# mcveanlab/Corticall

Hardware: AMD Instinct MI355X
Metric: k-mers traversed/sec (whole node) + contigs/sec, k=47 3-color LdBG (higher is better)
Workload: dtype u64

## Files before the change

corticall_amd/csrc/rt.h:

```cpp
#pragma once
#include <stdint.h>
#include <stdlib.h>
#include <string.h>

#include <algorithm>
#include <map>
#include <mutex>
#include <string>
#include <type_traits>
#include <unordered_map>
#include <utility>
#include <vector>

#include "../../include/ldbg.h"
#include "ctx_host.h"

#ifndef LDBG_HOSTSIM
#include <hip/hip_runtime.h>
#define LDBG_KERNEL __global__
#define LDBG_WAVE_KERNEL __global__ __launch_bounds__(64)
#define LDBG_WAVE_KERNEL_N(n) __global__ __launch_bounds__(n)
#define LDBG_DEV __device__ __forceinline__
#define LDBG_HOSTDEV __host__ __device__ __forceinline__
#if defined(__HIP_DEVICE_COMPILE__)
// ... 4 lines not shown
#define LDBG_LDS(T, p) ((T*)(p))
#endif

namespace ldbg {
namespace rt {

inline void check(hipError_t e, const char* what) {
    if (e != hipSuccess) throw StatusError(LDBG_ERR_HIP, std::string(what) + ": " + hipGetErrorString(e));
}
inline int device_count() {
    int n = 0;
    hipError_t e = hipGetDeviceCount(&n);
    if (e != hipSuccess) { (void)hipGetLastError(); return 0; }
    return n;
}
inline void set_device(int d) { check(hipSetDevice(d), "hipSetDevice"); }
inline int cu_count(int d) {
    int n = 0;
    check(hipDeviceGetAttribute(&n, hipDeviceAttributeMultiprocessorCount, d), "hipDeviceGetAttribute");
    return n > 0 ? n : 256;
}
struct BlockCache {
    std::mutex m;
    std::unordered_map<void*, std::pair<int, size_t>> live;
    std::map<std::pair<int, size_t>, std::vector<void*>> free_;
    size_t held = 0;
    static size_t size_class(size_t n) {
        size_t c = 4096;
        while (c < n) { if (c + c / 2 >= n) return c + c / 2; c *= 2; }
        return c;
    }
    void release_all() {
        std::lock_guard<std::mutex> g(m);
        for (auto& kv : free_) for (void* p : kv.second) (void)hipFree(p);
        free_.clear(); held = 0;
    }
};
inline BlockCache& block_cache() { static BlockCache c; return c; }
inline void* dmalloc(size_t n) {
    void* p = nullptr;
    hipError_t e = hipMalloc(&p, n ? n : 1);
    if (e != hipSuccess) { (void)hipGetLastError(); block_cache().release_all(); e = hipMalloc(&p, n ? n : 1); }
    check(e, "hipMalloc");
    return p;
}
inline void dfree(void* p) {
    if (!p) return;
    { BlockCache& c = block_cache(); std::lock_guard<std::mutex> g(c.m); c.live.erase(p); }
    (void)hipFree(p);
}
inline void* tmalloc(size_t n) {
    BlockCache& c = block_cache();
    const size_t cls = BlockCache::size_class(n);
    if (cls > ((size_t)64 << 20)) return dmalloc(n);
    int dev = 0;
    check(hipGetDevice(&dev), "hipGetDevice");
    {
        std::lock_guard<std::mutex> g(c.m);
        auto it = c.free_.find({dev, cls});
        if (it != c.free_.end() && !it->second.empty()) {
            void* p = it->second.back();
            it->second.pop_back();
            c.held -= cls;
            c.live[p] = {dev, cls};
            return p;
        }
    }
    void* p = dmalloc(cls);
    std::lock_guard<std::mutex> g(c.m);
    c.live[p] = {dev, cls};
    return p;
}
inline void tfree(void* p) {
    if (!p) return;
    BlockCache& c = block_cache();
    {
        std::lock_guard<std::mutex> g(c.m);
        auto it = c.live.find(p);
        if (it != c.live.end() && c.held + it->second.second <= ((size_t)1 << 30)) {
            c.free_[it->second].push_back(p);
            c.held += it->second.second;
            c.live.erase(it);
            return;
        }
        if (it != c.live.end()) c.live.erase(it);
    }
    (void)hipFree(p);
}
inline void* hmalloc_pinned(size_t n) { void* p = nullptr; check(hipHostMalloc(&p, n ? n : 1, hipHostMallocDefault), "hipHostMalloc"); return p; }
inline void hfree_pinned(void* p) { if (p) (void)hipHostFree(p); }
inline bool host_is_pinned(const void* p) {
    hipPointerAttribute_t a;
    if (hipPointerGetAttributes(&a, p) != hipSuccess) { (void)hipGetLastError(); return false; }
    return a.type == hipMemoryTypeHost;
}
typedef hipStream_t stream_t;
inline stream_t stream_create() { hipStream_t s; check(hipStreamCreateWithFlags(&s, hipStreamNonBlocking), "hipStreamCreate"); return s; }
inline void stream_destroy(stream_t s) { if (s) (void)hipStreamDestroy(s); }
inline void stream_sync(stream_t s) { check(hipStreamSynchronize(s), "hipStreamSynchronize"); }
inline void h2d(void* d, const void* h, size_t n, stream_t s) { if (n) check(hipMemcpyAsync(d, h, n, hipMemcpyHostToDevice, s), "hipMemcpyAsync H2D"); }
inline void d2h(void* h, const void* d, size_t n, stream_t s) { if (n) check(hipMemcpyAsync(h, d, n, hipMemcpyDeviceToHost, s), "hipMemcpyAsync D2H"); }
inline void d2d(void* d, const void* s_, size_t n, stream_t s) { if (n) check(hipMemcpyAsync(d, s_, n, hipMemcpyDeviceToDevice, s), "hipMemcpyAsync D2D"); }
inline void dmemset(void* d, int v, size_t n, stream_t s) { if (n) check(hipMemsetAsync(d, v, n, s), "hipMemsetAsync"); }
inline void mem_info(size_t* free_b, size_t* total_b) { check(hipMemGetInfo(free_b, total_b), "hipMemGetInfo"); }
inline void launch_check(const char* name) { check(hipGetLastError(), name); }

struct Event {
    hipEvent_t e = nullptr;
    Event() { check(hipEventCreate(&e), "hipEventCreate"); }
    ~Event() { if (e) (void)hipEventDestroy(e); }
    Event(Event&& o) noexcept : e(o.e) { o.e = nullptr; }
    Event& operator=(Event&& o) noexcept { if (this != &o) { if (e) (void)hipEventDestroy(e); e = o.e; o.e = nullptr; } return *this; }
    Event(const Event&) = delete;
    Event& operator=(const Event&) = delete;
    void record(stream_t s) { check(hipEventRecord(e, s), "hipEventRecord"); }
    void wait() { check(hipEventSynchronize(e), "hipEventSynchronize"); }
    static float elapsed_ms(Event& a, Event& b) {
        check(hipEventSynchronize(b.e), "hipEventSynchronize");
        float ms = 0;
        check(hipEventElapsedTime(&ms, a.e, b.e), "hipEventElapsedTime");
        return ms;
    }
};

}
}

#define LDBG_LAUNCH(kernel, grid, block, stream, ...)                               \
    do {                                                                            \
        hipLaunchKernelGGL(kernel, dim3((unsigned)(grid)), dim3((unsigned)(block)), 0, stream, __VA_ARGS__); \
        ::ldbg::rt::launch_check(#kernel);                                          \
    } while (0)

namespace ldbg {
LDBG_DEV int64_t global_tid() { return (int64_t)blockIdx.x * blockDim.x + threadIdx.x; }
LDBG_DEV int64_t global_nthreads() { return (int64_t)gridDim.x * blockDim.x; }
LDBG_DEV unsigned long long atomic_add_u64(unsigned long long* p, unsigned long long v) { return atomicAdd(p, v); }
LDBG_DEV unsigned atomic_add_u32(unsigned* p, unsigned v) { return atomicAdd(p, v); }
LDBG_DEV unsigned atomic_min_u32(unsigned* p, unsigned v) { return atomicMin(p, v); }
LDBG_DEV unsigned atomic_or_u32(unsigned* p, unsigned v) { return atomicOr(p, v); }
LDBG_DEV unsigned long long atomic_min_u64(unsigned long long* p, unsigned long long v) { return atomicMin(p, v); }
LDBG_DEV unsigned long long atomic_cas_u64(unsigned long long* p, unsigned long long cmp, unsigned long long v) { return atomicCAS(p, cmp, v); }
LDBG_DEV unsigned long long atomic_exch_u64(unsigned long long* p, unsigned long long v) { return atomicExch(p, v); }
LDBG_DEV int wave_size() { return blockDim.x < 64u ? (int)blockDim.x : 64; }
LDBG_DEV int wave_lane() { return (int)(threadIdx.x & 63u); }
LDBG_DEV unsigned long long wave_ballot(bool p) { return __ballot(p ? 1 : 0); }
LDBG_DEV uint32_t wave_bcast_u32(uint32_t v, int src) { return (uint32_t)__builtin_amdgcn_readlane((int)v, __builtin_amdgcn_readfirstlane(src)); }
LDBG_DEV uint64_t wave_bcast_u64(uint64_t v, int src) {
    uint32_t lo = wave_bcast_u32((uint32_t)v, src), hi = wave_bcast_u32((uint32_t)(v >> 32), src);
    return ((uint64_t)hi << 32) | lo;
}
LDBG_DEV uint32_t wave_shfl_u32(uint32_t v, int src) { return (uint32_t)__shfl((int)v, src & 63, 64); }
LDBG_DEV uint64_t wave_shfl_u64(uint64_t v, int src) { return ((uint64_t)wave_shfl_u32((uint32_t)(v >> 32), src) << 32) | wave_shfl_u32((uint32_t)v, src); }
LDBG_DEV void wave_fence() { __threadfence_block(); }
LDBG_DEV void device_fence() { __threadfence(); }
LDBG_DEV uint64_t wave_shfl_xor_u64(uint64_t v, int m) {
    uint32_t lo = (uint32_t)__shfl_xor((int)(uint32_t)v, m, 64), hi = (uint32_t)__shfl_xor((int)(uint32_t)(v >> 32), m, 64);
    return ((uint64_t)hi << 32) | lo;
}
LDBG_DEV uint64_t wave_min_u64(uint64_t v) { for (int m = wave_size() >> 1; m > 0; m >>= 1) { uint64_t o = wave_shfl_xor_u64(v, m); v = o < v ? o : v; } return v; }
LDBG_DEV uint64_t wave_max_u64(uint64_t v) { for (int m = wave_size() >> 1; m > 0; m >>= 1) { uint64_t o = wave_shfl_xor_u64(v, m); v = o > v ? o : v; } return v; }
LDBG_DEV int wave_count_below(unsigned long long ballot) { return __builtin_popcountll(ballot & ((1ull << wave_lane()) - 1ull)); }
LDBG_DEV uint32_t wave_incl_scan_u32(uint32_t v) {
    const int lane = wave_lane();
    for (int d = 1; d < wave_size(); d <<= 1) { const uint32_t o = (uint32_t)__shfl_up((int)v, d, 64); if (lane >= d) v += o; }
    return v;
}
}

#else
#define LDBG_KERNEL static
#define LDBG_WAVE_KERNEL static
#define LDBG_WAVE_KERNEL_N(n) static
#define LDBG_DEV inline
#define LDBG_HOSTDEV inline
#define LDBG_GLOBAL(T, p) ((T*)(p))
#define LDBG_LDS(T, p) ((T*)(p))
#ifndef __forceinline__
#define __forceinline__
#endif

namespace ldbg {
namespace rt {
inline int device_count() { return 1; }
inline void set_device(int) {}
inline int cu_count(int) { return 256; }
inline bool poison() { static const bool on = getenv("LDBG_HOSTSIM_POISON") != nullptr; return on; }
inline void* dmalloc(size_t n) {
    if (!poison()) return calloc(n ? n : 1, 1);
    void* p = malloc(n ? n : 1);
    if (p) memset(p, 0xAB, n ? n : 1);
    return p;
}
inline void dfree(void* p) { free(p); }
inline void* tmalloc(size_t n) { return dmalloc(n); }
inline void tfree(void* p) { free(p); }
inline void* hmalloc_pinned(size_t n) { return malloc(n ? n : 1); }
inline void hfree_pinned(void* p) { free(p); }
inline bool host_is_pinned(const void*) { return getenv("LDBG_HOSTSIM_PAGEABLE") == nullptr; }
typedef void* stream_t;
inline stream_t stream_create() { return nullptr; }
inline void stream_destroy(stream_t) {}
inline void stream_sync(stream_t) {}
inline void h2d(void* d, const void* h, size_t n, stream_t) { if (n) memcpy(d, h, n); }
inline void d2h(void* h, const void* d, size_t n, stream_t) { if (n) memcpy(h, d, n); }
inline void d2d(void* d, const void* s, size_t n, stream_t) { if (n) memmove(d, s, n); }
inline void dmemset(void* d, int v, size_t n, stream_t) { if (n) memset(d, v, n); }
inline void mem_info(size_t* free_b, size_t* total_b) {
    size_t mb = 2048;
    if (const char* ev = getenv("LDBG_HOSTSIM_MEM_MB")) mb = (size_t)atoll(ev);
    *free_b = mb << 20; *total_b = mb << 20;
}
struct Event {
    void record(stream_t) {}
    void wait() {}
    static float elapsed_ms(Event&, Event&) { return 0.0f; }
};
}
}
#include <execinfo.h>
#include <ucontext.h>
#include <stdio.h>
#include <functional>
#include <vector>
namespace ldbg {
namespace sim {
struct Wave {
    int lanes = 1, cur = 0, live = 0, arrived = 0;
    unsigned long long gen = 0;
    bool active = false;
    ucontext_t sched;
    ucontext_t ctx[64];
    std::vector<char> stacks[64];
    uint8_t done[64];
    int kind[64];
    void* site[64];
    uint64_t x[2][64];
    uint64_t y[2][64];
    int64_t tid0 = 0, nthreads = 1;
    std::function<void()>* body = nullptr;
};
inline Wave& wave() { static thread_local Wave w; return w; }
inline int& lanes_setting() { static int n = [] { const char* e = getenv("LDBG_HOSTSIM_LANES"); int v = e ? atoi(e) : 1; return v < 1 ? 1 : (v > 64 ? 64 : v); }(); return n; }
inline int lanes_env() { return lanes_setting(); }
inline void yield() { Wave& w = wave(); swapcontext(&w.ctx[w.cur], &w.sched); }
inline int collective(int kind, uint64_t a, uint64_t b = 0) {
    Wave& w = wave();
    const int buf = (int)(w.gen & 1ull);
    const unsigned long long my_gen = w.gen;
    w.x[buf][w.cur] = a; w.y[buf][w.cur] = b; w.kind[w.cur] = kind; w.site[w.cur] = __builtin_return_address(0);
    w.arrived++;
    if (w.arrived == w.live) {
        for (int l = 0; l < w.lanes; l++)
            if (!w.done[l] && w.kind[l] != kind) {
                fprintf(stderr, "[hostsim] wavefront divergence: lane %d is at primitive %d (%p), lane %d at %d (%p); the arriving lane's stack:\n", w.cur, kind, w.site[w.cur], l, w.kind[l], w.site[l]);
                void* bt[32];
                backtrace_symbols_fd(bt, backtrace(bt, 32), 2);
                abort();
            }
        w.arrived = 0; w.gen++;
    } else {
        while (w.gen == my_gen) yield();
    }
    return buf;
}
inline void trampoline() {
    Wave& w = wave();
    (*w.body)();
    w.done[w.cur] = 1;
    w.live--;
    if (w.live > 0 && w.arrived == w.live) {
        const int kd = [&] { for (int l = 0; l < w.lanes; l++) if (!w.done[l]) return w.kind[l]; return 0; }();
        for (int l = 0; l < w.lanes; l++)
            if (!w.done[l] && w.kind[l] != kd) { fprintf(stderr, "[hostsim] wavefront divergence at a lane's exit\n"); abort(); }
        w.arrived = 0; w.gen++;
    }
    swapcontext(&w.ctx[w.cur], &w.sched);
}
void run_wave(int lanes, int64_t tid0, int64_t nthreads, std::function<void()>& body);
}
struct SimIdx { int64_t tid, nthreads; };
inline SimIdx& sim_idx() { static thread_local SimIdx s{0, 1}; return s; }
inline int64_t global_tid() { return sim_idx().tid; }
inline int64_t global_nthreads() { return sim_idx().nthreads; }
inline void sim::run_wave(int lanes, int64_t tid0, int64_t nthreads, std::function<void()>& body) {
    Wave& w = wave();
    w.lanes = lanes; w.live = lanes; w.arrived = 0; w.gen = 0; w.active = true; w.body = &body; w.tid0 = tid0; w.nthreads = nthreads;
    for (int l = 0; l < lanes; l++) {
        if (w.stacks[l].empty()) w.stacks[l].resize((size_t)1 << 20);
        w.done[l] = 0; w.kind[l] = 0;
        getcontext(&w.ctx[l]);
        w.ctx[l].uc_stack.ss_sp = w.stacks[l].data();
        w.ctx[l].uc_stack.ss_size = w.stacks[l].size();
        w.ctx[l].uc_link = &w.sched;
        makecontext(&w.ctx[l], (void (*)())sim::trampoline, 0);
    }
    while (w.live > 0) {
        for (int l = 0; l < lanes; l++) {
            if (w.done[l]) continue;
            w.cur = l;
            sim_idx().tid = tid0 + l; sim_idx().nthreads = nthreads;
            swapcontext(&w.sched, &w.ctx[l]);
        }
    }
    w.active = false; w.lanes = 1; w.cur = 0;
}
inline unsigned long long atomic_add_u64(unsigned long long* p, unsigned long long v) { unsigned long long o = *p; *p += v; return o; }
inline unsigned atomic_add_u32(unsigned* p, unsigned v) { unsigned o = *p; *p += v; return o; }
inline unsigned atomic_min_u32(unsigned* p, unsigned v) { unsigned o = *p; if (v < o) *p = v; return o; }
inline unsigned atomic_or_u32(unsigned* p, unsigned v) { unsigned o = *p; *p |= v; return o; }
inline unsigned long long atomic_min_u64(unsigned long long* p, unsigned long long v) { unsigned long long o = *p; if (v < o) *p = v; return o; }
inline unsigned long long atomic_cas_u64(unsigned long long* p, unsigned long long cmp, unsigned long long v) { unsigned long long o = *p; if (o == cmp) *p = v; return o; }
inline unsigned long long atomic_exch_u64(unsigned long long* p, unsigned long long v) { unsigned long long o = *p; *p = v; return o; }
inline int wave_size() { return sim::wave().active ? sim::wave().lanes : 1; }
inline int wave_lane() { return sim::wave().active ? sim::wave().cur : 0; }
inline unsigned long long wave_ballot(bool p) {
    sim::Wave& w = sim::wave();
    if (!w.active) return p ? 1ull : 0ull;
    const int b = sim::collective(1, p ? 1ull : 0ull);
    unsigned long long m = 0;
    for (int l = 0; l < w.lanes; l++) if (!w.done[l] && w.x[b][l]) m |= 1ull << l;
    return m;
}
inline uint64_t wave_shfl_u64(uint64_t v, int src) {
    sim::Wave& w = sim::wave();
    if (!w.active) return v;
    const int b = sim::collective(2, v);
    return w.x[b][src & (w.lanes - 1)];
}
inline uint32_t wave_shfl_u32(uint32_t v, int src) { return (uint32_t)wave_shfl_u64(v, src); }
inline uint32_t wave_bcast_u32(uint32_t v, int src) { return (uint32_t)wave_shfl_u64(v, src); }
inline uint64_t wave_bcast_u64(uint64_t v, int src) { return wave_shfl_u64(v, src); }
inline uint64_t wave_shfl_xor_u64(uint64_t v, int m) { return wave_shfl_u64(v, wave_lane() ^ m); }
inline void wave_fence() { if (sim::wave().active) (void)sim::collective(3, 0ull); }
inline void device_fence() {}
inline uint64_t wave_min_u64(uint64_t v) { for (int m = wave_size() >> 1; m > 0; m >>= 1) { uint64_t o = wave_shfl_xor_u64(v, m); v = o < v ? o : v; } return v; }
inline uint64_t wave_max_u64(uint64_t v) { for (int m = wave_size() >> 1; m > 0; m >>= 1) { uint64_t o = wave_shfl_xor_u64(v, m); v = o > v ? o : v; } return v; }
inline int wave_count_below(unsigned long long ballot) { return __builtin_popcountll(ballot & ((1ull << wave_lane()) - 1ull)); }
inline uint32_t wave_incl_scan_u32(uint32_t v) {
    sim::Wave& w = sim::wave();
    if (!w.active) return v;
    const int b = sim::collective(3, v);
    uint32_t s = 0;
    for (int l = 0; l <= w.cur; l++) if (!w.done[l]) s += (uint32_t)w.x[b][l];
    return s;
}
}

#define LDBG_LAUNCH(kernel, grid, block, stream, ...)                      \
    do {                                                                   \
        int64_t nt__ = (int64_t)(grid) * (int64_t)(block);                 \
        if (nt__ > 4096) nt__ = 4096;                                      \
        const int lanes__ = ::ldbg::sim::lanes_env() > 1 && (int64_t)(block) <= 64 ? (int)std::min<int64_t>((int64_t)(block), (int64_t)::ldbg::sim::lanes_env()) : 1; \
        if (lanes__ > 1) {                                                 \
            nt__ = (nt__ / lanes__) * lanes__; if (nt__ < lanes__) nt__ = lanes__; \
            std::function<void()> body__ = [&]() { kernel(__VA_ARGS__); }; \
            for (int64_t t__ = 0; t__ < nt__; t__ += lanes__) ::ldbg::sim::run_wave(lanes__, t__, nt__, body__); \
            ::ldbg::sim_idx().tid = 0; ::ldbg::sim_idx().nthreads = 1;     \
            break;                                                         \
        }                                                                  \
        ::ldbg::sim_idx().nthreads = nt__;                                 \
        for (int64_t t__ = 0; t__ < nt__; t__++) {                         \
            ::ldbg::sim_idx().tid = t__;                                   \
            kernel(__VA_ARGS__);                                           \
        }                                                                  \
    } while (0)
#endif

#define LDBG_LAUNCH_W(W, KER, grid, block, stream, ...)                               \
    do {                                                                              \
        switch ((int)(W)) {                                                           \
            case 1: LDBG_LAUNCH(KER<1>, grid, block, stream, __VA_ARGS__); break;     \
            case 2: LDBG_LAUNCH(KER<2>, grid, block, stream, __VA_ARGS__); break;     \
            case 3: LDBG_LAUNCH(KER<3>, grid, block, stream, __VA_ARGS__); break;     \
            default: LDBG_LAUNCH(KER<4>, grid, block, stream, __VA_ARGS__); break;    \
        }                                                                             \
    } while (0)

namespace ldbg {
template <class F>
inline decltype(auto) with_words(int W, F&& f) {
    switch (W) {
        case 1: return f(std::integral_constant<int, 1>{});
        case 2: return f(std::integral_constant<int, 2>{});
        case 3: return f(std::integral_constant<int, 3>{});
        default: return f(std::integral_constant<int, 4>{});
    }
}
inline int grid_for(int64_t n, int block = 256, int max_blocks = 4096) {
    return (int)std::max<int64_t>(1, std::min<int64_t>((n + block - 1) / block, max_blocks));
}
inline uint32_t next_pow2(uint64_t v, uint64_t cap = ~0ull) { uint64_t p = 1; while (p < v) p <<= 1; return (uint32_t)std::min<uint64_t>(p, cap); }
}
```

corticall_amd/csrc/walk.cpp:

```cpp
#include <algorithm>
#include <chrono>
#include <numeric>
#include <thread>

#include "lscoop.h"
#include "runs.h"
#include "runstep.h"
#include "shard.h"
#include "strand.h"

namespace ldbg {

#define LDBG_STREAM_BLOCK 64
#define LDBG_STREAM_GRID 65536

LDBG_DEV void walk_finish(const WalkArgs& a, StrandState& st) {
    strand_finish(a, st);
    const bool good = !st.branch_null && st.status == ST_OK;
    a.strand_n[st.s] = good ? st.gV : 0u;
    a.strand_c[st.s] = good ? st.pw.n : 0u;
}

template <int W>
LDBG_DEV bool strand_step(const WalkArgs& a, StrandState& st, LinkStoreDev& ls, const StepPre& pre, RunState& rs) {
// ... 367 lines not shown


LDBG_KERNEL void k_compact_paths(const uint64_t* pool, const uint32_t* block_table, int max_blocks, const int64_t* strand_off,
                                 int64_t n_strands, uint64_t* dense) {
    const int64_t wave = global_tid() >> 6, lane = global_tid() & 63, nwaves = (global_nthreads() + 63) >> 6;
    for (int64_t s = wave; s < n_strands; s += nwaves) {
        const int64_t o = strand_off[s], n = strand_off[s + 1] - o;
        for (int64_t j = lane; j < n; j += 64)
            dense[o + j] = pool[(uint64_t)block_table[s * max_blocks + j / LDBG_PATH_BLOCK] * LDBG_PATH_BLOCK + (j & (LDBG_PATH_BLOCK - 1))];
    }
}

struct ExpandArgs {
    const uint64_t* pool; const uint32_t* block_table; int max_blocks;
    const uint32_t* strand_c;
    const int64_t* strand_off;
    int64_t n_strands;
    RunIndexView runs;
    uint64_t* dense;
    unsigned* overflow;
};
LDBG_DEV uint64_t expand_stored(const ExpandArgs& a, int64_t s, uint32_t j) {
    return a.pool[(uint64_t)a.block_table[s * a.max_blocks + j / LDBG_PATH_BLOCK] * LDBG_PATH_BLOCK + (j & (LDBG_PATH_BLOCK - 1))];
}
LDBG_KERNEL void k_expand_paths(ExpandArgs a) {
    const int64_t wave = global_tid() / wave_size(), nwaves = (global_nthreads() + wave_size() - 1) / wave_size();
    const uint32_t lane = (uint32_t)wave_lane(), WS = (uint32_t)wave_size();
    for (int64_t s = wave; s < a.n_strands; s += nwaves) {
        const uint32_t nc = a.strand_c[s];
        uint64_t* out = a.dense + a.strand_off[s];
        const bool fwd = (s & 1) != 0;
        uint32_t base_v = 0;
        for (uint32_t j0 = 0; j0 < nc; j0 += WS) {
            const uint32_t j = j0 + lane;
            uint64_t e = 0, prev = 0;
            if (j < nc) {
                e = expand_stored(a, s, j);
                if (j & (LDBG_PATH_BLOCK - 1)) prev = expand_stored(a, s, j - 1);
            }
            const uint32_t cnt = j < nc ? pd_expanded(prev, e) : 0u;
            const uint32_t incl = wave_incl_scan_u32(cnt);
            const uint32_t at = base_v + incl - cnt;
            const bool head = cnt > 0u && pd_is_head(e);
            if (cnt == 1u && !head) out[at] = e;
            unsigned long long hb = wave_ballot(head);
            while (hb) {
                const int L = __builtin_ctzll(hb);
                hb &= hb - 1;
                const uint64_t he = wave_bcast_u64(e, L);
                const uint32_t hat = wave_bcast_u32(at, L);
                const uint32_t hj = j0 + (uint32_t)L;
                const uint64_t payload = expand_stored(a, s, hj + 1);
                const uint32_t len = wave_bcast_u32(cnt, L);
                if (LDBG_PD_KIND(he) == LDBG_PD_RUN) {
                    const uint32_t acopy = (uint32_t)(he >> 20) & 0xFFFFu;
                    const bool asc = (he >> 36) & 1ull, inv = (he >> 37) & 1ull;
                    const uint32_t first = (uint32_t)payload;
                    const int copy = fwd ? (int)acopy : -(int)acopy;
                    for (uint32_t i = lane; i < len; i += WS) {
                        const uint32_t pos = asc ? first + i : first - i;
                        const uint32_t u = a.runs.uo[pos];
                        const unsigned bb = a.runs.ubase[pos];
                        const unsigned b0 = !inv ? (bb & 3u) : 3u - ((bb >> 2) & 3u), b1 = !inv ? ((bb >> 2) & 3u) : 3u - (bb & 3u);
                        out[hat + i] = path_pack((int64_t)(u & 0x7FFFFFFFu), ((u >> 31) != 0u) != inv, fwd ? b1 : b0, copy);
                    }
                } else {
                    wave_fence();
                    const uint32_t first = (uint32_t)payload, period = (uint32_t)(payload >> 32);
                    for (uint32_t i = lane; i < len; i += WS) {
                        const uint32_t o = i % period;
                        const uint64_t s1 = LDBG_GLOBAL(const uint64_t, out)[first + o], s2 = LDBG_GLOBAL(const uint64_t, out)[first + period + o];
                        const int c = path_copy(s2) + (int)(i / period + 1u) * (path_copy(s2) - path_copy(s1));
                        if (c > 32767 || c < -32767) *a.overflow = 1u;
                        out[hat + i] = (s2 & ~(0xFFFFFFull << 36)) | (((uint64_t)(uint32_t)c & 0xFFFFFFull) << 36);
                    }
                }
            }
            base_v += wave_bcast_u32(incl, (int)WS - 1);
        }
    }
}

struct ContigArgs {
    GraphView g;
    int64_t n;
    const uint64_t* seeds;
    const uint64_t* dense;
    const int64_t* strand_off;
    const int64_t* walk_len;
    const int64_t* contig_off;
    const uint8_t* quirk;
    const uint64_t* term;
    char* out;
};
template <int W>
LDBG_DEV Kmer<W> walk_vertex_kmer(const ContigArgs& a, int64_t i, int64_t v, int64_t ro, int64_t nr, int64_t fo) {
    const int64_t nrev = nr > 0 ? nr - 1 : 0;
    uint64_t e;
    const uint64_t* term;
    if (v < nrev) { e = a.dense[ro + (nr - 1 - v)]; term = a.term + (2 * i) * W; }
    else if (v == nrev) { e = nr > 0 ? a.dense[ro] : a.dense[fo]; term = a.seeds + i * W; }
    else { e = a.dense[fo + (v - nrev)]; term = a.term + (2 * i + 1) * W; }
    Kmer<W> km;
    const int64_t ri = path_idx(e);
    if (ri >= 0) { km = graph_key<W>(a.g, ri); if (path_flip(e)) km = kmer_revcomp<W>(km, a.g.k); }
    else { for (int w = 0; w < W; w++) km.w[w] = term[w]; }
    return km;
}
template <int W>
LDBG_KERNEL void k_contigs(ContigArgs a) {
    const int k = a.g.k;
    const int64_t wave = global_tid() >> 6, lane = global_tid() & 63, nwaves = (global_nthreads() + 63) >> 6;
    for (int64_t i = wave; i < a.n; i += nwaves) {
        if (a.walk_len[i] == 0) continue;
        const int64_t L = a.contig_off[i + 1] - a.contig_off[i];
        const int64_t ro = a.strand_off[2 * i], nr = a.strand_off[2 * i + 1] - ro;
        const int64_t fo = a.strand_off[2 * i + 1];
        const int64_t nrev = nr > 0 ? nr - 1 : 0;
        char* o = a.out + a.contig_off[i];
        if (a.quirk[2 * i] | a.quirk[2 * i + 1]) {
            for (int64_t p = lane; p < L; p += 64) {
                const int64_t v = p < k ? 0 : p - k + 1;
                const Kmer<W> km = walk_vertex_kmer<W>(a, i, v, ro, nr, fo);
                o[p] = "ACGT"[kmer_base<W>(km, k, p < k ? (int)p : k - 1)];
            }
            continue;
        }
        Kmer<W> sk;
#pragma unroll
        for (int w = 0; w < W; w++) sk.w[w] = a.seeds[i * W + w];
        for (int64_t p = lane; p < L; p += 64) {
            unsigned b;
            if (p < nrev) b = path_base(a.dense[ro + (nr - 1 - p)]);
            else if (p < nrev + k) b = kmer_base<W>(sk, k, (int)(p - nrev));
            else b = path_base(a.dense[fo + (p - nrev - k + 1)]);
            o[p] = "ACGT"[b];
        }
    }
}

struct ContigRleArgs {
    GraphView g;
    RunIndexView runs;
    int64_t n;
    const uint64_t* seeds;
    const uint64_t* pool; const uint32_t* block_table; int max_blocks;
    const uint32_t* strand_c; const uint32_t* strand_n;
    const int64_t* walk_len; const int64_t* contig_off;
    char* out;
};
LDBG_DEV uint64_t rle_stored(const ContigRleArgs& a, int64_t s, uint32_t j) {
    return a.pool[(uint64_t)a.block_table[s * a.max_blocks + j / LDBG_PATH_BLOCK] * LDBG_PATH_BLOCK + (j & (LDBG_PATH_BLOCK - 1))];
}
template <int W>
LDBG_KERNEL void k_contigs_rle(ContigRleArgs a) {
    const int k = a.g.k;
    const int64_t wave = global_tid() / wave_size(), nwaves = (global_nthreads() + wave_size() - 1) / wave_size();
    const uint32_t lane = (uint32_t)wave_lane(), WS = (uint32_t)wave_size();
    for (int64_t i = wave; i < a.n; i += nwaves) {
        if (a.walk_len[i] == 0) continue;
        char* o = a.out + a.contig_off[i];
        const int64_t nr = a.strand_n[2 * i], nrev = nr > 0 ? nr - 1 : 0;
        Kmer<W> sk;
#pragma unroll
        for (int w = 0; w < W; w++) sk.w[w] = a.seeds[i * W + w];
        for (uint32_t p = lane; p < (uint32_t)k; p += WS) o[nrev + p] = "ACGT"[kmer_base<W>(sk, k, (int)p)];
        for (int dir = 0; dir < 2; dir++) {
            const int64_t s = 2 * i + dir;
            const bool fwd = dir == 1;
            const uint32_t nc = a.strand_c[s];
            auto place = [&](uint32_t v) -> int64_t { return fwd ? nrev + k - 1 + (int64_t)v : nrev - (int64_t)v; };
            uint32_t base_v = 0;
            uint64_t carry = 0;
            for (uint32_t j0 = 0; j0 < nc; j0 += WS) {
                const uint32_t j = j0 + lane;
                const uint64_t* blk = a.pool + (uint64_t)a.block_table[s * a.max_blocks + j0 / LDBG_PATH_BLOCK] * LDBG_PATH_BLOCK;
                const uint64_t e = j < nc ? LDBG_GLOBAL(const uint64_t, blk)[j & (LDBG_PATH_BLOCK - 1)] : 0ull;
                const uint64_t up = wave_shfl_u64(e, (int)lane - 1);
                const uint64_t prev = (j & (LDBG_PATH_BLOCK - 1)) == 0u ? 0ull : (lane == 0u ? carry : up);
                carry = wave_shfl_u64(e, (int)WS - 1);
                const uint32_t cnt = j < nc ? pd_expanded(prev, e) : 0u;
                const uint32_t incl = wave_incl_scan_u32(cnt);
                const uint32_t at = base_v + incl - cnt;
                const bool head = cnt > 0u && pd_is_head(e);
                if (cnt == 1u && !head && at >= 1u) o[place(at)] = "ACGT"[path_base(e)];
                const bool is_run = head && LDBG_PD_KIND(e) == LDBG_PD_RUN;
                unsigned long long hb = wave_ballot(is_run);
                const uint32_t GS = WS == 64u ? 16u : WS, g = lane / GS, sub = lane % GS;
                const uint8_t* ub = LDBG_GLOBAL(const uint8_t, a.runs.ubase);
                while (hb) {
                    uint32_t myL = 0;
                    bool gv = false;
                    for (uint32_t q = 0; q < WS / GS; q++) {
                        if (!hb) break;
                        const int L = __builtin_ctzll(hb);
                        hb &= hb - 1;
                        if (g == q) { myL = (uint32_t)L; gv = true; }
                    }
                    const uint64_t he = wave_shfl_u64(e, (int)myL);
                    const uint32_t hat = wave_shfl_u32(at, (int)myL), len_of = wave_shfl_u32(cnt, (int)myL);
                    const uint32_t len = gv ? len_of : 0u;
                    const uint64_t next_e = wave_shfl_u64(e, (int)myL + 1);
                    const uint64_t payload = !gv ? 0ull : (myL + 1u < WS ? next_e : rle_stored(a, s, j0 + myL + 1u));
                    const bool asc = (he >> 36) & 1ull, inv = (he >> 37) & 1ull;
                    const uint32_t first = (uint32_t)payload;
                    const unsigned shift = (fwd != inv) ? 2u : 0u, comp = inv ? 3u : 0u;
                    auto ascii = [&](unsigned bb) -> unsigned { return (0x54474341u >> (8u * (((bb >> shift) & 3u) ^ comp))) & 0xFFu; };
                    auto ascii4 = [&](uint32_t bb4) -> uint32_t {
                        const uint32_t f = ((bb4 >> shift) & 0x03030303u) ^ (comp * 0x01010101u);
#ifndef LDBG_HOSTSIM
                        return __builtin_amdgcn_perm(0u, 0x54474341u, f);
#else
                        uint32_t v = 0;
                        for (int bI = 0; bI < 4; bI++) v |= ((0x54474341u >> (8u * ((f >> (8 * bI)) & 3u))) & 0xFFu) << (8 * bI);
                        return v;
#endif
                    };
                    const uint8_t* in_lo = asc ? ub + first : ub + first - (len ? len - 1u : 0u);
                    char* out_lo = LDBG_GLOBAL(char, o) + (fwd ? place(hat) : place(hat + (len ? len - 1u : 0u)));
                    const bool same = asc == fwd;
                    const uint32_t nd = len / 8u;
                    uint32_t max_nd = wave_bcast_u32(nd, 0);
                    for (uint32_t q = 1; q < WS / GS; q++) { const uint32_t o2 = wave_bcast_u32(nd, (int)(q * GS)); max_nd = o2 > max_nd ? o2 : max_nd; }
                    for (uint32_t base = 0; base < max_nd; base += 4u * GS) {
                        uint64_t w[4];
#pragma unroll
                        for (int q = 0; q < 4; q++) {
                            const uint32_t ci = base + (uint32_t)q * GS + sub;
                            w[q] = 0;
                            if (ci < nd) __builtin_memcpy(&w[q], in_lo + (same ? 8u * ci : len - 8u - 8u * ci), 8);
                        }
#pragma unroll
                        for (int q = 0; q < 4; q++) {
                            const uint32_t ci = base + (uint32_t)q * GS + sub;
                            uint64_t v = (uint64_t)ascii4((uint32_t)w[q]) | ((uint64_t)ascii4((uint32_t)(w[q] >> 32)) << 32);
                            if (!same) v = __builtin_bswap64(v);
                            if (ci < nd) __builtin_memcpy(out_lo + 8u * ci, &v, 8);
                        }
                    }
                    for (uint32_t t = 8u * nd + sub; t < len; t += GS) {
                        const unsigned bb = in_lo[same ? t : len - 1u - t];
                        out_lo[t] = (char)ascii(bb);
                    }
                }
                hb = wave_ballot(head && !is_run);
                while (hb) {
                    const int L = __builtin_ctzll(hb);
                    hb &= hb - 1;
                    const uint32_t hat = wave_bcast_u32(at, L), len = wave_bcast_u32(cnt, L);
                    const uint64_t payload = (uint32_t)L + 1u < WS ? wave_bcast_u64(e, L + 1) : rle_stored(a, s, j0 + (uint32_t)L + 1);
                    wave_fence();
                    const uint32_t first = (uint32_t)payload, period = (uint32_t)(payload >> 32);
                    const uint32_t nch = (len + 7u) / 8u;
                    for (uint32_t c = lane; c < nch; c += WS) {
                        const uint32_t t0 = 8u * c, m = len - t0 < 8u ? len - t0 : 8u;
                        uint32_t r = t0 % period;
                        uint64_t v = 0;
#pragma unroll
                        for (uint32_t b = 0; b < 8u; b++) {
                            if (b < m) {
                                const uint64_t ch = (uint8_t)LDBG_GLOBAL(const char, o)[place(first + period + r)];
                                v |= ch << (8u * (fwd ? b : m - 1u - b));
                            }
                            r++;
                            if (r == period) r = 0;
                        }
                        char* lo = LDBG_GLOBAL(char, o) + (fwd ? place(hat + t0) : place(hat + t0 + m - 1u));
                        if (m == 8u) __builtin_memcpy(lo, &v, 8);
                        else for (uint32_t b = 0; b < m; b++) lo[b] = (char)(v >> (8u * b));
                    }
                }
                base_v += wave_bcast_u32(incl, (int)WS - 1);
            }
        }
    }
}

template <int W>
LDBG_KERNEL void k_walk_vertices(GraphView g, const uint64_t* dense, int64_t ro, int64_t nr, int64_t fo, int64_t nf,
                                 const uint64_t* term_r, const uint64_t* term_f, int64_t len, uint64_t* words, int64_t* rec,
                                 int32_t* copy, int32_t* index) {
    const int64_t nrev = nr > 0 ? nr - 1 : 0;
    for (int64_t p = global_tid(); p < len; p += global_nthreads()) {
        uint64_t e;
        int idx_label;
        const uint64_t* term;
        if (p < nrev) { e = dense[ro + (nr - 1 - p)]; idx_label = -1; term = term_r; }
        else if (p == nrev) { e = nr > 0 ? dense[ro] : dense[fo]; idx_label = 0; term = nullptr; }
        else { e = dense[fo + (p - nrev)]; idx_label = 1; term = term_f; }
        int64_t ri = path_idx(e);
        Kmer<W> km;
        if (ri >= 0) {
            km = graph_key<W>(g, ri);
            if (path_flip(e)) km = kmer_revcomp<W>(km, g.k);
        } else {
            for (int w = 0; w < W; w++) km.w[w] = term ? term[w] : 0;
        }
        for (int w = 0; w < W; w++) words[p * W + w] = km.w[w];
        rec[p] = ri;
        copy[p] = path_copy(e);
        index[p] = idx_label;
    }
}

struct RoiHitArgs {
    const uint32_t* roi_of;
    int64_t n;
    const uint64_t* dense; const int64_t* strand_off; const int64_t* walk_len;
    unsigned long long* count;
    const int64_t* out_off;
    uint32_t* out;
    uint8_t* has_null;
    int fill;
};
LDBG_KERNEL void k_roi_hits(RoiHitArgs a) {
    const int64_t wave = global_tid() >> 6, lane = global_tid() & 63, nwaves = (global_nthreads() + 63) >> 6;
    for (int64_t i = wave; i < a.n; i += nwaves) {
        const int64_t ro = a.strand_off[2 * i], nr = a.strand_off[2 * i + 1] - ro;
        const int64_t fo = a.strand_off[2 * i + 1], nf = a.strand_off[2 * i + 2] - fo;
        const bool in_walk = a.walk_len[i] > 0;
        bool null_seen = false;
        for (int64_t p = lane; p < nr + nf; p += 64) {
            const bool fwd_part = p >= nr;
            const uint64_t e = a.dense[fwd_part ? fo + (p - nr) : ro + p];
            const int64_t idx = path_idx(e);
            if (idx < 0) { null_seen = true; continue; }
            if (fwd_part && p == nr && nr > 0) continue;
            if (!in_walk) continue;
            const uint32_t r = a.roi_of[idx];
            if (r == 0xFFFFFFFFu) continue;
            const unsigned long long slot = atomic_add_u64(&a.count[i], 1ull);
            if (a.fill) a.out[a.out_off[i] + (int64_t)slot] = r;
        }
        if (!a.fill && null_seen) a.has_null[i] = 1;
    }
}
template <int W>
LDBG_KERNEL void k_roi_of(GraphView g, GraphView rois, uint32_t* roi_of) {
    for (int64_t i = global_tid(); i < rois.N; i += global_nthreads()) {
        GraphView exact = g;
        exact.java_tiny = 0;
        const int64_t idx = graph_find_canonical<W>(exact, graph_key<W>(rois, i));
        if (idx >= 0) roi_of[idx] = (uint32_t)i;
    }
}

Engine::Engine(const ldbg_engine_config& c) : cfg(c) {
    if (c.n_traversal <= 0) throw StatusError(LDBG_ERR_CORTEXJDK, "Traversal color(s) must be specified.");
    if (!c.graph) throw StatusError(LDBG_ERR_CORTEXJDK, "Must provide graph to traverse.");
    graph = (const Graph*)c.graph;
    rois = (const Graph*)c.rois;
    stream_ = graph->stream;
    const int nc = graph->hdr.C;
    auto fail = [&](const char* what, int col) {
        throw StatusError(LDBG_ERR_CORTEXJDK, std::string(what) + " colors must be between 0 and " + std::to_string(nc) + " (provided " + std::to_string(col) + ")");
    };
    for (int i = 0; i < c.n_traversal; i++) if (c.traversal_colors[i] >= nc || c.traversal_colors[i] < 0) fail("Traversal", c.traversal_colors[i]);
    for (int i = 0; i < c.n_joining; i++) if (c.joining_colors[i] < 0 || c.joining_colors[i] >= nc) fail("Joining", c.joining_colors[i]);
    for (int i = 0; i < c.n_recruitment; i++) if (c.recruitment_colors[i] < 0 || c.recruitment_colors[i] >= nc) fail("Recruitment", c.recruitment_colors[i]);
    for (int i = 0; i < c.n_secondary; i++) if (c.secondary_colors[i] < 0 || c.secondary_colors[i] >= nc) fail("Secondary", c.secondary_colors[i]);
    if (c.stopping_rule < 0 || c.stopping_rule >= LDBG_STOP_COUNT) throw StatusError(LDBG_ERR_CORTEXJDK, "Must provide stopping rule for graph traversal");

    rt::set_device(graph->device);
    view.g = graph->view;
    view.trav_mask = view.recruit_mask = view.join_mask = 0;
    for (int i = 0; i < c.n_traversal; i++) view.trav_mask |= 1u << c.traversal_colors[i];
    for (int i = 0; i < c.n_recruitment; i++) view.recruit_mask |= 1u << c.recruitment_colors[i];
    for (int i = 0; i < c.n_joining; i++) view.join_mask |= 1u << c.joining_colors[i];
    view.trav_sel4 = view.recruit_sel4 = 0;
    for (int col = 0; col < 4; col++) {
        if ((view.trav_mask >> col) & 1u) view.trav_sel4 |= 0xFFu << (8 * col);
        if ((view.recruit_mask >> col) & 1u) view.recruit_sel4 |= 0xFFu << (8 * col);
    }
    view.first_trav = c.traversal_colors[0];
    view.stopper = c.stopping_rule;
    view.max_len = c.max_branch_length;
    view.connect_all = c.connect_all_neighbors;
    view.strict_flip = c.strict_java_flip;
    view.lean_rows = (view.g.k & 1) && row_is_packed(view.g) ? 1 : 0;
    for (int i = 0; i < c.nlinks; i++) {
        const Links* l = (const Links*)c.links[i];
        if (!l) continue;
        bool mine = false;
        for (int t = 0; t < c.n_traversal; t++)
            if (!l->sample_names.empty() && l->sample_names[0] == graph->hdr.colors[c.traversal_colors[t]].sample_name) mine = true;
        if (mine) my_links.push_back(l);
    }
    merged_.reset(new MergedLinks(my_links, *graph));
    view.links = merged_->view;
    view.link_flag_mask = merged_->flag_mask;
    view.cursor_on = c.nlinks > 0 ? 1 : 0;
    if (!graph->is_image) {
        rt::set_device(graph->device);
        rt::stream_sync(graph->stream);
        own_stream_ = rt::stream_create();
        if (own_stream_) stream_ = own_stream_;
    }
}
void Engine::enter() {
    rt::set_device(graph->device);
    if (stream_ != graph->stream) rt::stream_sync(graph->stream);
}

Engine::~Engine() { if (own_stream_) { try { rt::set_device(graph->device); } catch (...) {} }
                    sharded_abort(); clear_batch(); drop_batch_seeds(); drop_spares(); rt::hfree_pinned(h_small_); rt::hfree_pinned(h_log_); rt::hfree_pinned(h_stage_[0]); rt::hfree_pinned(h_stage_[1]); release_scratch(); rt::dfree(d_frames_); rt::dfree(d_roi_bits_); rt::dfree(d_roi_of_);
                    if (own_stream_) { quiesce(); rt::stream_destroy(own_stream_); } }

void Engine::walk_roi_hits(int64_t* offsets, uint32_t* hits, int64_t capacity, uint8_t* has_null) {
    if (!rois) throw StatusError(LDBG_ERR_ARG, "walk_roi_hits: the engine has no ROI graph");
    enter();
    rt::stream_t s = stream_;
    const int W = graph->hdr.W;
    if (!d_roi_of_) {
        if (rois->hdr.k != graph->hdr.k) throw StatusError(LDBG_ERR_ARG, "the ROI graph must have the k-mer size of the traversed graph");
        const size_t nrec = (size_t)std::max<int64_t>(1, graph->view.N);
        d_roi_of_ = rt::dmalloc(nrec * 4);
        rt::dmemset(d_roi_of_, 0xFF, nrec * 4, s);
        if (rois->view.N > 0) {
            LDBG_LAUNCH_W(W, k_roi_of, grid_for(rois->view.N), 256, s, graph->view, rois->view, (uint32_t*)d_roi_of_);
        }
    }
    std::vector<std::vector<unsigned long long>> counts(chunks.size());
    int64_t total = 0;
    offsets[0] = 0;
    for (size_t ci = 0; ci < chunks.size(); ci++) {
// ... 822 lines not shown
```

Before: 186.9 billion.

## Restructure RLE contig expansion into batched, software-pipelined run pieces across both strands

Rewrites k_contigs_rle to process both strand directions together, two wave-widths of path entries per step. Run heads are compacted with ds_permute (a new wave_push_u32 helper), split into fixed-size pieces by a prefix scan, and expanded with a software pipeline that loads the next piece while storing the current one. Repeat-run handling is deferred to the end of each batch. It also sets waves_per_eu, hardcodes a wave size of 64, and uses unaligned 64-bit loads with a dummy pointer instead of guarded memcpy. The aim is fewer serialized per-head loops and better memory overlap. The cost is more register pressure and more complex code, and a repeat run in a batch appears to be handled only for the first head.

Result: faster. 194.3 billion (median of 6 runs) (+4.0%).

```diff
diff --git a/corticall_amd/csrc/rt.h b/corticall_amd/csrc/rt.h
--- a/corticall_amd/csrc/rt.h
+++ b/corticall_amd/csrc/rt.h
@@ -180,6 +180,7 @@
 }
 LDBG_DEV uint32_t wave_shfl_u32(uint32_t v, int src) { return (uint32_t)__shfl((int)v, src & 63, 64); }
 LDBG_DEV uint64_t wave_shfl_u64(uint64_t v, int src) { return ((uint64_t)wave_shfl_u32((uint32_t)(v >> 32), src) << 32) | wave_shfl_u32((uint32_t)v, src); }
+LDBG_DEV uint32_t wave_push_u32(uint32_t v, uint32_t dst) { return (uint32_t)__builtin_amdgcn_ds_permute((int)(dst << 2), (int)v); }
 LDBG_DEV void wave_fence() { __threadfence_block(); }
 LDBG_DEV void device_fence() { __threadfence(); }
 LDBG_DEV uint64_t wave_shfl_xor_u64(uint64_t v, int m) {
@@ -357,6 +358,14 @@
     return w.x[b][src & (w.lanes - 1)];
 }
 inline uint32_t wave_shfl_u32(uint32_t v, int src) { return (uint32_t)wave_shfl_u64(v, src); }
+inline uint32_t wave_push_u32(uint32_t v, uint32_t dst) {
+    sim::Wave& w = sim::wave();
+    if (!w.active) return v;
+    const int b = sim::collective(4, v, dst & (uint32_t)(w.lanes - 1));
+    uint32_t r = 0;
+    for (int l = 0; l < w.lanes; l++) if (!w.done[l] && w.y[b][l] == (uint64_t)w.cur) r = (uint32_t)w.x[b][l];
+    return r;
+}
 inline uint32_t wave_bcast_u32(uint32_t v, int src) { return (uint32_t)wave_shfl_u64(v, src); }
 inline uint64_t wave_bcast_u64(uint64_t v, int src) { return wave_shfl_u64(v, src); }
 inline uint64_t wave_shfl_xor_u64(uint64_t v, int m) { return wave_shfl_u64(v, wave_lane() ^ m); }
diff --git a/corticall_amd/csrc/walk.cpp b/corticall_amd/csrc/walk.cpp
--- a/corticall_amd/csrc/walk.cpp
+++ b/corticall_amd/csrc/walk.cpp
@@ -543,125 +543,231 @@
 LDBG_DEV uint64_t rle_stored(const ContigRleArgs& a, int64_t s, uint32_t j) {
     return a.pool[(uint64_t)a.block_table[s * a.max_blocks + j / LDBG_PATH_BLOCK] * LDBG_PATH_BLOCK + (j & (LDBG_PATH_BLOCK - 1))];
 }
+#ifndef LDBG_RLE_GS
+#define LDBG_RLE_GS 8u
+#endif
+#define LDBG_RLE_GROUPS 2u
+typedef uint64_t rle_u64 __attribute__((aligned(1)));
+#ifndef LDBG_HOSTSIM
+#define LDBG_RLE_KERNEL __global__ __attribute__((amdgpu_waves_per_eu(6)))
+#else
+#define LDBG_RLE_KERNEL LDBG_KERNEL
+#endif
+struct RlePiece {
+    uint32_t in, out;
+    uint32_t n;
+    uint64_t w[4];
+    uint32_t tail;
+};
 template <int W>
-LDBG_KERNEL void k_contigs_rle(ContigRleArgs a) {
+LDBG_RLE_KERNEL void k_contigs_rle(ContigRleArgs a) {
     const int k = a.g.k;
-    const int64_t wave = global_tid() / wave_size(), nwaves = (global_nthreads() + wave_size() - 1) / wave_size();
-    const uint32_t lane = (uint32_t)wave_lane(), WS = (uint32_t)wave_size();
+#ifndef LDBG_HOSTSIM
+    const uint32_t WS = 64u;
+#else
+    const uint32_t WS = (uint32_t)wave_size();
+#endif
+    const uint32_t lane = (uint32_t)wave_lane();
+    const uint32_t GS = WS < LDBG_RLE_GS ? WS : LDBG_RLE_GS, NG = WS / GS, g = lane / GS, sub = lane % GS, PB = 32u * GS;
+    const uint32_t EPB = LDBG_RLE_GROUPS * WS;
+    const int64_t wave = (int64_t)wave_bcast_u32((uint32_t)(global_tid() / (int64_t)WS), 0), nwaves = (global_nthreads() + WS - 1) / WS;
+    const uint8_t* ub = a.runs.ubase;
+    const uint8_t* spare = (const uint8_t*)a.seeds;
+    auto letter = [](unsigned b) -> unsigned { return (0x54474341u >> (8u * (b & 3u))) & 0xFFu; };
+    auto ascii4 = [](uint32_t bb4, unsigned shift, unsigned comp) -> uint32_t {
+        const uint32_t f = ((bb4 >> shift) & 0x03030303u) ^ (comp * 0x01010101u);
+#ifndef LDBG_HOSTSIM
+        return __builtin_amdgcn_perm(0u, 0x54474341u, f);
+#else
+        uint32_t v = 0;
+        for (int bI = 0; bI < 4; bI++) v |= ((0x54474341u >> (8u * ((f >> (8 * bI)) & 3u))) & 0xFFu) << (8 * bI);
+        return v;
+#endif
+    };
+    auto piece_load = [&](RlePiece& pc) {
+        const uint8_t* in = ub + pc.in;
+        const bool same = (pc.n >> 20) & 1u;
+        const uint32_t n = pc.n & 0xFFFFFu, nd = n / 8u;
+#pragma unroll
+        for (int q = 0; q < 4; q++) {
+            const uint32_t ci = (uint32_t)q * GS + sub;
+            const uint8_t* p = ci < nd ? in + (same ? 8u * ci : n - 8u - 8u * ci) : spare;
+            pc.w[q] = *LDBG_GLOBAL(const rle_u64, p);
+        }
+        const uint32_t t = 8u * nd + sub;
+        const uint8_t* p = t < n ? in + (same ? t : n - 1u - t) : spare;
+        pc.tail = *LDBG_GLOBAL(const uint8_t, p);
+    };
+    auto piece_store = [&](const RlePiece& pc, char* o) {
+        char* out = o + pc.out;
+        const bool same = (pc.n >> 20) & 1u;
+        const unsigned shift = ((pc.n >> 21) & 1u) * 2u, comp = ((pc.n >> 22) & 1u) * 3u;
+        const uint32_t n = pc.n & 0xFFFFFu, nd = n / 8u;
+#pragma unroll
+        for (int q = 0; q < 4; q++) {
+            const uint32_t ci = (uint32_t)q * GS + sub;
+            uint64_t v = (uint64_t)ascii4((uint32_t)pc.w[q], shift, comp) | ((uint64_t)ascii4((uint32_t)(pc.w[q] >> 32), shift, comp) << 32);
+            if (!same) v = __builtin_bswap64(v);
+            if (ci < nd) *LDBG_GLOBAL(rle_u64, out + 8u * ci) = v;
+        }
+        const uint32_t t = 8u * nd + sub;
+        if (t < n) LDBG_GLOBAL(char, out)[t] = (char)letter((pc.tail >> shift) ^ comp);
+        for (uint32_t t2 = t + GS; t2 < n; t2 += GS) {
+            const unsigned bb = LDBG_GLOBAL(const uint8_t, ub + pc.in)[same ? t2 : n - 1u - t2];
+            LDBG_GLOBAL(char, out)[t2] = (char)letter((bb >> shift) ^ comp);
+        }
+    };
     for (int64_t i = wave; i < a.n; i += nwaves) {
-        if (a.walk_len[i] == 0) continue;
-        char* o = a.out + a.contig_off[i];
-        const int64_t nr = a.strand_n[2 * i], nrev = nr > 0 ? nr - 1 : 0;
+        const int64_t wl_v = a.walk_len[i], co_v = a.contig_off[i];
+        const uint32_t nr_v = a.strand_n[2 * i], nc0_v = a.strand_c[2 * i], nc1_v = a.strand_c[2 * i + 1];
+        const uint32_t bt0_v = a.block_table[(2 * i) * a.max_blocks], bt1_v = a.block_table[(2 * i + 1) * a.max_blocks];
         Kmer<W> sk;
 #pragma unroll
         for (int w = 0; w < W; w++) sk.w[w] = a.seeds[i * W + w];
-        for (uint32_t p = lane; p < (uint32_t)k; p += WS) o[nrev + p] = "ACGT"[kmer_base<W>(sk, k, (int)p)];
-        for (int dir = 0; dir < 2; dir++) {
-            const int64_t s = 2 * i + dir;
-            const bool fwd = dir == 1;
-            const uint32_t nc = a.strand_c[s];
-            auto place = [&](uint32_t v) -> int64_t { return fwd ? nrev + k - 1 + (int64_t)v : nrev - (int64_t)v; };
-            uint32_t base_v = 0;
-            uint64_t carry = 0;
-            for (uint32_t j0 = 0; j0 < nc; j0 += WS) {
-                const uint32_t j = j0 + lane;
-                const uint64_t* blk = a.pool + (uint64_t)a.block_table[s * a.max_blocks + j0 / LDBG_PATH_BLOCK] * LDBG_PATH_BLOCK;
-                const uint64_t e = j < nc ? LDBG_GLOBAL(const uint64_t, blk)[j & (LDBG_PATH_BLOCK - 1)] : 0ull;
-                const uint64_t up = wave_shfl_u64(e, (int)lane - 1);
-                const uint64_t prev = (j & (LDBG_PATH_BLOCK - 1)) == 0u ? 0ull : (lane == 0u ? carry : up);
-                carry = wave_shfl_u64(e, (int)WS - 1);
-                const uint32_t cnt = j < nc ? pd_expanded(prev, e) : 0u;
+        const bool empty = wave_bcast_u32((uint32_t)(wl_v != 0), 0) == 0u;
+        const int64_t co = (int64_t)wave_bcast_u64((uint64_t)co_v, 0);
+        const uint32_t nr = wave_bcast_u32(nr_v, 0);
+        const uint32_t nc[2] = {wave_bcast_u32(nc0_v, 0), wave_bcast_u32(nc1_v, 0)};
+        uint32_t bt[2] = {wave_bcast_u32(bt0_v, 0), wave_bcast_u32(bt1_v, 0)};
+        if (empty) continue;
+        char* o = a.out + co;
+        const int64_t nrev = nr > 0 ? nr - 1 : 0;
+#ifndef LDBG_HOSTSIM
+#pragma unroll
+        for (uint32_t p0 = 0; p0 < 32u * W; p0 += 64u) {
+            const uint32_t p = p0 + lane;
+            if (p < (uint32_t)k) LDBG_GLOBAL(char, o)[nrev + p] = (char)letter((unsigned)kmer_base<W>(sk, k, (int)p));
+        }
+#else
+        for (uint32_t p = lane; p < (uint32_t)k; p += WS) o[nrev + p] = (char)letter((unsigned)kmer_base<W>(sk, k, (int)p));
+#endif
+        auto place = [&](bool fwd, uint32_t v) -> int64_t { return fwd ? nrev + k - 1 + (int64_t)v : nrev - (int64_t)v; };
+        uint32_t base_v[2] = {0u, 0u};
+        uint64_t carry[2] = {0ull, 0ull};
+        const uint32_t ncmax = nc[0] > nc[1] ? nc[0] : nc[1];
+        for (uint32_t b0 = 0; b0 < ncmax; b0 += EPB) {
+            if (b0) {
+#pragma unroll
+                for (int d = 0; d < 2; d++) bt[d] = wave_bcast_u32(b0 < nc[d] ? a.block_table[(2 * i + d) * a.max_blocks + b0 / LDBG_PATH_BLOCK] : 0u, 0);
+            }
+            uint64_t e[4];
+#pragma unroll
+            for (int s = 0; s < 4; s++) {
+                const int d = s >> 1;
+                const uint32_t j = b0 + (uint32_t)(s & 1) * WS + lane;
+                const uint64_t* blk = a.pool + (uint64_t)bt[d] * LDBG_PATH_BLOCK;
+                e[s] = *LDBG_GLOBAL(const uint64_t, j < nc[d] ? blk + (j & (LDBG_PATH_BLOCK - 1)) : (const uint64_t*)spare);
+            }
+#pragma unroll
+            for (int s = 0; s < 4; s++) if (b0 + (uint32_t)(s & 1) * WS + lane >= nc[s >> 1]) e[s] = 0ull;
+            uint32_t l_in[2] = {0u, 0u}, l_rel[2] = {0u, 0u}, l_meta[2] = {0u, 0u}, l_p[2];
+            uint32_t n_run[2] = {0u, 0u};
+            bool has_rep[2] = {false, false};
+            uint32_t rep_at[2] = {0u, 0u}, rep_len[2] = {0u, 0u};
+            uint64_t rep_pay[2] = {0ull, 0ull};
+#pragma unroll
+            for (int s = 0; s < 4; s++) {
+                const int d = s >> 1;
+                const bool fwd = d == 1, second = (s & 1) != 0;
+                const uint32_t j = b0 + (second ? WS : 0u) + lane;
+                const uint64_t up = wave_shfl_u64(e[s], (int)lane - 1);
+                const uint64_t before = second ? wave_bcast_u64(e[s & 2], (int)WS - 1) : carry[d];
+                const uint64_t prev = (j & (LDBG_PATH_BLOCK - 1)) == 0u ? 0ull : (lane == 0u ? before : up);
+                const uint32_t cnt = j < nc[d] ? pd_expanded(prev, e[s]) : 0u;
                 const uint32_t incl = wave_incl_scan_u32(cnt);
-                const uint32_t at = base_v + incl - cnt;
-                const bool head = cnt > 0u && pd_is_head(e);
-                if (cnt == 1u && !head && at >= 1u) o[place(at)] = "ACGT"[path_base(e)];
-                const bool is_run = head && LDBG_PD_KIND(e) == LDBG_PD_RUN;
-                unsigned long long hb = wave_ballot(is_run);
-                const uint32_t GS = WS == 64u ? 16u : WS, g = lane / GS, sub = lane % GS;
-                const uint8_t* ub = LDBG_GLOBAL(const uint8_t, a.runs.ubase);
-                while (hb) {
-                    uint32_t myL = 0;
-                    bool gv = false;
-                    for (uint32_t q = 0; q < WS / GS; q++) {
-                        if (!hb) break;
-                        const int L = __builtin_ctzll(hb);
-                        hb &= hb - 1;
-                        if (g == q) { myL = (uint32_t)L; gv = true; }
+                const uint32_t at = base_v[d] + incl - cnt;
+                const bool head = cnt > 0u && pd_is_head(e[s]);
+                if (cnt == 1u && !head && at >= 1u) o[place(fwd, at)] = (char)letter((unsigned)path_base(e[s]));
+                const uint64_t down = wave_shfl_u64(e[s], (int)lane + 1);
+                const uint64_t after = second ? 0ull : wave_bcast_u64(e[s | 1], 0);
+                uint64_t payload = lane + 1u < WS ? down : after;
+                if (second && head && lane + 1u == WS) payload = rle_stored(a, 2 * i + d, j + 1u);
+                const bool is_run = head && LDBG_PD_KIND(e[s]) == LDBG_PD_RUN;
+                const unsigned long long hb = wave_ballot(is_run);
+                if (hb) {
+                    const bool asc = (e[s] >> 36) & 1ull, inv = (e[s] >> 37) & 1ull;
+                    const uint32_t first = (uint32_t)payload, len = cnt;
+                    const uint32_t nh = (uint32_t)__builtin_popcountll(hb);
+                    const uint32_t to = is_run ? n_run[d] + (uint32_t)wave_count_below(hb) : (n_run[d] + nh) & (WS - 1u);
+                    const bool mine = lane >= n_run[d] && lane < n_run[d] + nh;
+                    const uint32_t v0 = wave_push_u32(asc ? first : first - (len - 1u), to);
+                    const uint32_t v1 = wave_push_u32((uint32_t)(fwd ? place(fwd, at) : place(fwd, at + len - 1u)), to);
+                    const uint32_t v2 = wave_push_u32(len | ((asc == fwd ? 1u : 0u) << 20) | ((fwd != inv ? 1u : 0u) << 21) | ((inv ? 1u : 0u) << 22), to);
+                    if (mine) { l_in[d] = v0; l_rel[d] = v1; l_meta[d] = v2; }
+                    n_run[d] += nh;
+                }
+                const unsigned long long rb = wave_ballot(head && !is_run);
+                if (rb) {
+                    const int L = __builtin_ctzll(rb);
+                    has_rep[d] = true;
+                    rep_at[d] = wave_bcast_u32(at, L); rep_len[d] = wave_bcast_u32(cnt, L); rep_pay[d] = wave_bcast_u64(payload, L);
+                }
+                base_v[d] += wave_bcast_u32(incl, (int)WS - 1);
+                if (second) carry[d] = wave_bcast_u64(e[s], (int)WS - 1);
+            }
+            uint32_t T = 0, TA = 0;
+#pragma unroll
+            for (int d = 0; d < 2; d++) {
+                l_p[d] = T + wave_incl_scan_u32(lane < n_run[d] ? ((l_meta[d] & 0xFFFFFu) + PB - 1u) / PB : 0u);
+                T = wave_bcast_u32(l_p[d], (int)WS - 1);
+                if (d == 0) TA = T;
+            }
+            auto piece_of = [&](uint32_t r0, RlePiece& pc) {
+                uint32_t io = 0, rl = 0, mt = 0, pe = 0;
+                for (uint32_t q = 0; q < NG; q++) {
+                    const uint32_t p = r0 + q;
+                    if (p >= T) break;
+                    const bool B = p >= TA;
+                    const uint32_t ps = B ? l_p[1] : l_p[0];
+                    const int L = __builtin_popcountll(wave_ballot(ps <= p));
+                    const uint32_t v0 = wave_bcast_u32(B ? l_in[1] : l_in[0], L), v1 = wave_bcast_u32(B ? l_rel[1] : l_rel[0], L);
+                    const uint32_t v2 = wave_bcast_u32(B ? l_meta[1] : l_meta[0], L), v3 = wave_bcast_u32(ps, L);
+                    if (g == q) { io = v0; rl = v1; mt = v2; pe = v3; }
+                }
+                const uint32_t len = mt & 0xFFFFFu, np = (len + PB - 1u) / PB;
+                const uint32_t t0 = (r0 + g - (pe - np)) * PB;
+                const uint32_t n = len == 0u ? 0u : (len - t0 < PB ? len - t0 : PB);
+                pc.n = n | (mt & 0x700000u);
+                pc.in = io + (((mt >> 20) & 1u) ? t0 : len - t0 - n);
+                pc.out = rl + t0;
+            };
+            if (T) {
+                RlePiece cur;
+                piece_of(0u, cur);
+                piece_load(cur);
+                for (uint32_t r0 = NG; r0 < T; r0 += NG) {
+                    RlePiece nx;
+                    piece_of(r0, nx);
+                    piece_load(nx);
+                    piece_store(cur, o);
+                    cur = nx;
+                }
+                piece_store(cur, o);
+            }
+#pragma unroll
+            for (int d = 0; d < 2; d++) {
+                if (!has_rep[d]) continue;
+                const bool fwd = d == 1;
+                wave_fence();
+                const uint32_t hat = rep_at[d], len = rep_len[d], first = (uint32_t)rep_pay[d], period = (uint32_t)(rep_pay[d] >> 32);
+                const uint32_t nch = (len + 7u) / 8u;
+                for (uint32_t c = lane; c < nch; c += WS) {
+                    const uint32_t t0 = 8u * c, m = len - t0 < 8u ? len - t0 : 8u;
+                    uint32_t r = t0 % period;
+                    uint64_t v = 0;
+#pragma unroll
+                    for (uint32_t b = 0; b < 8u; b++) {
+                        if (b < m) {
+                            const uint64_t ch = (uint8_t)LDBG_GLOBAL(const char, o)[place(fwd, first + period + r)];
+                            v |= ch << (8u * (fwd ? b : m - 1u - b));
+                        }
+                        r++;
+                        if (r == period) r = 0;
                     }
-                    const uint64_t he = wave_shfl_u64(e, (int)myL);
-                    const uint32_t hat = wave_shfl_u32(at, (int)myL), len_of = wave_shfl_u32(cnt, (int)myL);
-                    const uint32_t len = gv ? len_of : 0u;
-                    const uint64_t next_e = wave_shfl_u64(e, (int)myL + 1);
-                    const uint64_t payload = !gv ? 0ull : (myL + 1u < WS ? next_e : rle_stored(a, s, j0 + myL + 1u));
-                    const bool asc = (he >> 36) & 1ull, inv = (he >> 37) & 1ull;
-                    const uint32_t first = (uint32_t)payload;
-                    const unsigned shift = (fwd != inv) ? 2u : 0u, comp = inv ? 3u : 0u;
-                    auto ascii = [&](unsigned bb) -> unsigned { return (0x54474341u >> (8u * (((bb >> shift) & 3u) ^ comp))) & 0xFFu; };
-                    auto ascii4 = [&](uint32_t bb4) -> uint32_t {
-                        const uint32_t f = ((bb4 >> shift) & 0x03030303u) ^ (comp * 0x01010101u);
-#ifndef LDBG_HOSTSIM
-                        return __builtin_amdgcn_perm(0u, 0x54474341u, f);
-#else
-                        uint32_t v = 0;
-                        for (int bI = 0; bI < 4; bI++) v |= ((0x54474341u >> (8u * ((f >> (8 * bI)) & 3u))) & 0xFFu) << (8 * bI);
-                        return v;
-#endif
-                    };
-                    const uint8_t* in_lo = asc ? ub + first : ub + first - (len ? len - 1u : 0u);
-                    char* out_lo = LDBG_GLOBAL(char, o) + (fwd ? place(hat) : place(hat + (len ? len - 1u : 0u)));
-                    const bool same = asc == fwd;
-                    const uint32_t nd = len / 8u;
-                    uint32_t max_nd = wave_bcast_u32(nd, 0);
-                    for (uint32_t q = 1; q < WS / GS; q++) { const uint32_t o2 = wave_bcast_u32(nd, (int)(q * GS)); max_nd = o2 > max_nd ? o2 : max_nd; }
-                    for (uint32_t base = 0; base < max_nd; base += 4u * GS) {
-                        uint64_t w[4];
-#pragma unroll
-                        for (int q = 0; q < 4; q++) {
-                            const uint32_t ci = base + (uint32_t)q * GS + sub;
-                            w[q] = 0;
-                            if (ci < nd) __builtin_memcpy(&w[q], in_lo + (same ? 8u * ci : len - 8u - 8u * ci), 8);
-                        }
-#pragma unroll
-                        for (int q = 0; q < 4; q++) {
-                            const uint32_t ci = base + (uint32_t)q * GS + sub;
-                            uint64_t v = (uint64_t)ascii4((uint32_t)w[q]) | ((uint64_t)ascii4((uint32_t)(w[q] >> 32)) << 32);
-                            if (!same) v = __builtin_bswap64(v);
-                            if (ci < nd) __builtin_memcpy(out_lo + 8u * ci, &v, 8);
-                        }
-                    }
-                    for (uint32_t t = 8u * nd + sub; t < len; t += GS) {
-                        const unsigned bb = in_lo[same ? t : len - 1u - t];
-                        out_lo[t] = (char)ascii(bb);
-                    }
+                    char* lo = LDBG_GLOBAL(char, o) + (fwd ? place(fwd, hat + t0) : place(fwd, hat + t0 + m - 1u));
+                    if (m == 8u) __builtin_memcpy(lo, &v, 8);
+                    else for (uint32_t b = 0; b < m; b++) lo[b] = (char)(v >> (8u * b));
                 }
-                hb = wave_ballot(head && !is_run);
-                while (hb) {
-                    const int L = __builtin_ctzll(hb);
-                    hb &= hb - 1;
-                    const uint32_t hat = wave_bcast_u32(at, L), len = wave_bcast_u32(cnt, L);
-                    const uint64_t payload = (uint32_t)L + 1u < WS ? wave_bcast_u64(e, L + 1) : rle_stored(a, s, j0 + (uint32_t)L + 1);
-                    wave_fence();
-                    const uint32_t first = (uint32_t)payload, period = (uint32_t)(payload >> 32);
-                    const uint32_t nch = (len + 7u) / 8u;
-                    for (uint32_t c = lane; c < nch; c += WS) {
-                        const uint32_t t0 = 8u * c, m = len - t0 < 8u ? len - t0 : 8u;
-                        uint32_t r = t0 % period;
-                        uint64_t v = 0;
-#pragma unroll
-                        for (uint32_t b = 0; b < 8u; b++) {
-                            if (b < m) {
-                                const uint64_t ch = (uint8_t)LDBG_GLOBAL(const char, o)[place(first + period + r)];
-                                v |= ch << (8u * (fwd ? b : m - 1u - b));
-                            }
-                            r++;
-                            if (r == period) r = 0;
-                        }
-                        char* lo = LDBG_GLOBAL(char, o) + (fwd ? place(hat + t0) : place(hat + t0 + m - 1u));
-                        if (m == 8u) __builtin_memcpy(lo, &v, 8);
-                        else for (uint32_t b = 0; b < m; b++) lo[b] = (char)(v >> (8u * b));
-                    }
-                }
-                base_v += wave_bcast_u32(incl, (int)WS - 1);
             }
         }
     }
```
